# AMReX-Fluids/IAMR

Measured on AMD Instinct MI355X. Metric: cells-advanced/sec, higher is better.
Workload: dtype f64; 1 GPU; TaylorGreen 3D single level, one 256^3 box per GPU in a 1x1x1 arrangement (256x256x256 cells), periodic, nu=1e-4 cfl=0.7 Godunov_PLM be_cn_theta=0.5, full NavierStokes::advance per step

## Files before the change

iamr_amd/csrc/cabi.hip:

```cpp
#include "../../include/iamrx.h"
#include "operators.h"
#include "launch.h"
#include "amrns.h"
#include <string>
#include <cstring>
#include <vector>
#include <map>

using namespace iamrx;

struct iamrx_layout_s { LayoutP p; };
struct iamrx_mf_s { MultiFab mf; };

static thread_local std::string g_err;

#define IAMRX_TRY try {
#define IAMRX_CATCH                                                   \
    return 0; }                                                       \
    catch (const std::exception& e) { g_err = e.what(); return 1; }   \
    catch (...) { g_err = "unknown error"; return 2; }

static Geometry to_geom(const iamrx_geom* g)
{
    Geometry r;
// ... 102 lines not shown
            o[2] = cd.src_fab >= 0 ? local[cd.src_fab] : -1;
            o[3] = cd.dst_fab >= 0 ? local[cd.dst_fab] : -1;
            for (int d = 0; d < 3; ++d) { o[4 + d] = cd.region.lo[d]; o[7 + d] = cd.region.hi[d]; o[10 + d] = cd.shift[d]; }
            o[13] = (int)cd.buf_off; o[14] = 0; o[15] = 0;
        }
        ++n;
    };
    for (auto& cd : plan.local) emit(0, -1, cd);
    for (auto& kv : peers) {
        for (auto& cd : kv.second.pack) emit(1, kv.first, cd);
        for (auto& cd : kv.second.unpack) emit(2, kv.first, cd);
    }
    *ndesc = n;
    IAMRX_CATCH
}

int iamrx_host_abec_smoother_plan(int nboxes, const int* lo_hi, const iamrx_geom* g, const int lobc[3], const int hibc[3], int maxorder, int ncomp,
                                  int coef, int has_a, int has_cf, int finest, const int ngrow[4], int out[12])
{
    IAMRX_TRY
    if (nboxes < 1 || coef < 0 || coef > 2) throw Error("iamrx_host_abec_smoother_plan: at least one box; coef is 0 (stored), 1 (density) or 2 (uniform)");
    std::vector<BoxD> b(nboxes);
    AbecLevel lv;
    for (int i = 0; i < nboxes; ++i)
        for (int d = 0; d < 3; ++d) { b[i].lo[d] = lo_hi[6 * i + d]; b[i].hi[d] = lo_hi[6 * i + 3 + d]; lv.max_len[d] = std::max(lv.max_len[d], b[i].len(d)); }
    const DomainBC bc = to_bc(lobc, hibc, maxorder);
    lv.boxes = &b; lv.nlocal = nboxes; lv.ncomp = ncomp;
    lv.phi_ngrow = ngrow[0]; lv.rhs_ngrow = ngrow[1]; lv.sig_ngrow = ngrow[2]; lv.a_ngrow = ngrow[3];
    lv.sig = coef == 1; lv.b_uniform = coef == 2; lv.has_a = has_a != 0; lv.nbc = 1; lv.bcs = &bc; lv.has_cf = has_cf != 0; lv.finest = finest != 0;
    const AbecSmoothPlan p = abec_smooth_plan(to_geom(g), lv);
    const AbecColourForm& f = p.colour;
    const int v[12] = {(int)p.path, p.nw, p.nbr_splits, p.zero_first, (int)f.kernel, f.mode, f.np, f.maintain, f.allcf, f.wrap, f.walls_inkernel, f.zero_ok};
    std::copy(v, v + 12, out);
    IAMRX_CATCH
}

int iamrx_host_nodal_smoother_plan(int nboxes, const int* lo_hi, const iamrx_geom* g, const int lobc[3], const int hibc[3], int has_mask,
                                   int nodal_smoother, int bottom_smoother_only, int device_bottom, int nodal_sweeps, int coarsest, const int ngrow[2],
                                   int out[11])
{
    IAMRX_TRY
    if (nboxes < 1) throw Error("iamrx_host_nodal_smoother_plan: at least one box");
    std::vector<BoxD> b(nboxes);
    NodalLevel lv;
    for (int i = 0; i < nboxes; ++i)
        for (int d = 0; d < 3; ++d) { b[i].lo[d] = lo_hi[6 * i + d]; b[i].hi[d] = lo_hi[6 * i + 3 + d]; lv.max_len[d] = std::max(lv.max_len[d], b[i].len(d)); }
    DomainBC bc = to_bc(lobc, hibc, 2);
    for (int d = 0; d < 3; ++d) { if (bc.lo[d] == lo_inflow) bc.lo[d] = lo_neumann; if (bc.hi[d] == lo_inflow) bc.hi[d] = lo_neumann; }
    lv.boxes = &b; lv.nlocal = nboxes; lv.bc = &bc;
    lv.cor_ngrow = ngrow[0]; lv.rhs_ngrow = ngrow[1];
    lv.has_mask = has_mask != 0;
    lv.nodal_smoother = nodal_smoother; lv.bottom_smoother_only = bottom_smoother_only; lv.device_bottom = device_bottom; lv.nodal_sweeps = nodal_sweeps;
    lv.coarsest = coarsest != 0;
    const NodalSmoothPlan p = nodal_smooth_plan(to_geom(g), lv);
    const int v[11] = {(int)p.path, p.ngrow, p.wrap, p.refl, p.images, p.written_first, p.zero_start, p.par_fill, p.splits, (int)p.bottom, p.sweeps};
    std::copy(v, v + 11, out);
    IAMRX_CATCH
}

static hipEvent_t g_ev0 = nullptr, g_ev1 = nullptr;
int iamrx_timer_start(void)
{
    IAMRX_TRY
    if (!g_ev0) { IAMRX_HIP_CHECK(hipEventCreate(&g_ev0)); IAMRX_HIP_CHECK(hipEventCreate(&g_ev1)); }
    IAMRX_HIP_CHECK(hipEventRecord(g_ev0, Context::get().stream));
    IAMRX_CATCH
// ... 1463 lines not shown
```

iamr_amd/csrc/kernels.h:

```cpp
#pragma once
#include "core.h"
#include "mf.h"

namespace iamrx {

void launch_fill(double* p, size_t n, double v, hipStream_t s);
void launch_copy_plan(const CopyDesc* d, int nd, long maxpts, const FabD* src, const FabD* dst, int scomp, int dcomp, int nc, hipStream_t s, bool add = false);
void launch_pack(const CopyDesc* d, int nd, long maxpts, const FabD* src, double* buf, long pts_total, int scomp, int nc, hipStream_t s);
void launch_unpack(const CopyDesc* d, int nd, long maxpts, const FabD* dst, const double* buf, long pts_total, int dcomp, int nc, hipStream_t s, bool add = false);
void launch_copy_plan_w(const CopyDesc* d, const int2* w, int nw, const FabD* src, const FabD* dst, int scomp, int dcomp, int nc, hipStream_t s, bool add);
void launch_pack_w(const CopyDesc* d, const int2* w, int nw, const FabD* src, double* buf, long pts_total, int scomp, int nc, hipStream_t s);
void launch_unpack_w(const CopyDesc* d, const int2* w, int nw, const FabD* dst, const double* buf, long pts_total, int dcomp, int nc, hipStream_t s, bool add);
double reduce_norm0(const MultiFab& mf, int comp, int nc, int ng, bool global = false);
void reduce_norm0_comps(const MultiFab& mf, int comp, int nc, int ng, double* out, bool global = false);
void reduce_minmax(const MultiFab& mf, int comp, int ng, double& mn, double& mx, bool global = true);
double reduce_sum_unique(const MultiFab& mf, int comp, const Geometry& g, bool global = false);
void reduce_sum_integrated(const MultiFab& S, int rho_comp, int trac_comp, const MultiFab* cov, double out[3]);
void reduce_dots(int nout, const MultiFab* const* x, const MultiFab* const* y, int comp, int nc, const Geometry& g, double* out, bool local = false);
void reduce_dots_dev(int nout, const MultiFab* const* x, const MultiFab* const* y, int comp, int nc, const Geometry& g, double* d_out, bool local = false);
enum { PROBE_NODAL_GS4 = 0, PROBE_ABEC_GSRB = 1, PROBE_GOD_Z = 2, PROBE_PRED_Z = 3, PROBE_COUNT = 4 };
void kernel_probe_start(int which, long min_points, int stride);
void kernel_probe_stop(int which, double* total_ms, long* launches);
void kernel_probes_pause(bool on);
bool kernel_probe_begin(int which, long points);
// ... 51 lines not shown
    const DomainBC* bcs = nullptr;
    bool has_cf = false;
    bool finest = true;
};
AbecLevel abec_level(const AbecCoef& c, const MultiFab& phi, int rhs_ngrow, int nbc, const DomainBC* bcs, bool has_cf = false, bool finest = true);
struct AbecColourForm {
    enum Kernel { GENERAL, GSRB1, GSRB2, GSRB2_PER_COMP } kernel = GENERAL;
    int mode = 0;
    int np = 1;
    bool gen_mc = false;
    int gen_mode = 0;
    bool has_cf = false, maintain = false, allcf = false;
    bool wrap = false;
    bool walls_inkernel = false;
    bool zero_ok = false;
};
struct AbecSmoothPlan {
    enum Path { COLOUR, RB_BOX, RB_CF, RB_NBR, FUSED_SHELL } path = COLOUR;
    AbecColourForm colour;
    int nw = 16;
    bool nbr_splits = false;
    bool zero_first = false;
    int ncomp = 1, phi_ngrow = 1, rhs_ngrow = 0;
    bool sweep_kernel() const { return path == RB_BOX || path == RB_CF || path == RB_NBR; }
    bool made_for(const MultiFab& phi, const MultiFab& rhs) const { return phi.ncomp == ncomp && phi.ngrow == phi_ngrow && rhs.ngrow == rhs_ngrow; }
};
AbecSmoothPlan abec_smooth_plan(const Geometry& g, const AbecLevel& lv);
AbecColourForm abec_colour_form(const Geometry& g, const AbecLevel& lv, bool wrap = false, bool walls_inkernel = false);
void abec_gsrb(const Geometry& g, const AbecCoef& c, const AbecColourForm& f, MultiFab& phi, const MultiFab& rhs, int redblack, double omega,
               const DomainBC* bcs, int nbc, bool shell_only = false, bool phi_is_zero = false, const MultiFab* cfm = nullptr, const CfTab* cftab = nullptr);
bool abec_tail_ok(const Geometry& gF, const Layout& lF, const Geometry& gC, const Layout& lC, const AbecCoef& cF, const DomainBC* bcs, int nbc, int ncomp);
void abec_tail_solve(const Geometry& gF, const AbecCoef& cF, MultiFab& corF, const MultiFab& resF, const Geometry& gC, const AbecCoef& cC,
                     const DomainBC& bc, bool singular, double eps_rel, int maxiter, int nub, int nuf, int nu1, int nu2, double omega, int* d_iters);
bool abec_residual_reads_no_ghosts(const Geometry& g, const AbecCoef& c, const MultiFab& out, const MultiFab& phi, const MultiFab& rhs, bool restrict_form);
bool abec_resid_restrict_ok(const AbecCoef& c, const MultiFab& phi, const MultiFab& rhs);
void abec_resid_restrict(const Geometry& g, const AbecCoef& c, MultiFab& crse, const MultiFab& phi, const MultiFab& rhs);
void abec_gsrb_rb(const Geometry& g, const AbecCoef& c, const AbecSmoothPlan& p, const MultiFab& pin, MultiFab& pout, const MultiFab& rhs, double omega,
                  bool zero, const DomainBC* bcs = nullptr, int nbc = 0, const CfTab* cf = nullptr, bool acc = false);
void abec_gsrb_rb_nbr(const Geometry& g, const AbecCoef& c, const AbecSmoothPlan& p, MultiFab& pin, MultiFab& pout, const MultiFab& rhs, double omega,
                      bool zero, const DomainBC* bcs, int nbc, int sel = 0, hipStream_t on = nullptr, bool acc = false);
bool abec_gsrb_rb_ok(const Geometry& g, const AbecCoef& c, const MultiFab& phi, int nbc, const DomainBC* bcs = nullptr);
bool abec_gsrb_rb_cf_ok(const Geometry& g, const AbecCoef& c, const MultiFab& phi);
bool abec_gsrb_rb_nbr_ok(const Geometry& g, const AbecCoef& c, const MultiFab& phi, const MultiFab& rhs, int nbc, const DomainBC* bcs);
bool abec_gsrb_rb_nbr_level_ok(const Geometry& g, const Layout& l, int ncomp, bool sig_form, bool has_a, int nbc, const DomainBC* bcs);
void abec_gsrb_fused(const Geometry& g, const AbecCoef& c, const MultiFab& phi_in, MultiFab& phi_out, const MultiFab& rhs, double omega,
                     const DomainBC* bcs, int nbc);
void abec_residual(const Geometry& g, const AbecCoef& c, MultiFab& out, const MultiFab& phi, const MultiFab* rhs, double* norm_out = nullptr);
bool abec_bottom_device_ok(const Geometry& g, const Layout& l, const DomainBC* bcs, int nbc, int ncomp, bool cf = false);
void abec_bottom_solve(const Geometry& g, const AbecCoef& c, MultiFab& cor, const MultiFab& res, const DomainBC& bc, bool singular,
                       double eps_rel, int maxiter, int nub, int nuf, double omega, int* d_iters, const CfTab* cftab = nullptr);
void abec_apply_domain_bc(const Geometry& g, MultiFab& phi, const DomainBC& bc, bool inhomog, const MultiFab* bcval, int comp0 = 0, int ncomp = -1);
void abec_apply_domain_bc_percomp(const Geometry& g, MultiFab& phi, const DomainBC* bcs, int ncomp, bool inhomog, const MultiFab* bcval);
void cc_restrict(MultiFab& crse, const MultiFab& fine);
void cc_prolong_add(MultiFab& fine, const MultiFab& crse);
void face_avgdown(MultiFab& crse, const MultiFab& fine, int dir);
void abec_flux(const Geometry& g, const AbecCoef& c, const MultiFab& phi, MultiFab* const flux[3], MultiFab* const add_to[3]);
void mac_rhs(const Geometry& g, MultiFab& rhs, const MultiFab* const umac[3], const MultiFab* S);
void mac_bcoef(MultiFab* const b[3], const MultiFab& rho, int rho_comp, double scale);
void mac_divergence(const Geometry& g, MultiFab& div, const MultiFab* const umac[3]);

void godunov_extrap_vel_to_faces(const Geometry& g, const MultiFab& vel, const MultiFab* force, MultiFab* const umac[3],
                                 double dt, const BCRec* bc, bool use_forces_in_trans, int scheme = 0);
void godunov_compute_aofs(const Geometry& g, MultiFab& aofs, int acomp, const MultiFab& S, int ncomp, const MultiFab* force,
                          const MultiFab* divu, MultiFab* const umac[3], const int* iconserv, double dt, const BCRec* bc,
                          bool is_velocity, bool use_forces_in_trans, MultiFab* const edge_out[3], MultiFab* const flux_out[3], int scheme = 0);

// ... 73 lines not shown
```

iamr_amd/csrc/mlmg.h:

```cpp
#pragma once
#include <functional>
#include "mf.h"
#include "kernels.h"
#include <vector>
#include <memory>

namespace iamrx {

inline bool mg_stalled_at_floor(const std::vector<double>& hist, double r0, double target, bool fast)
{
    const size_t n = hist.size();
    if (n == 0 || !(hist[n - 1] <= 10.0 * target)) return false;
    if (n >= 4 && hist[n - 1] > 0.9 * hist[n - 4]) return true;
    if (!fast || n < 2) return false;
    const double last = hist[n - 1] / hist[n - 2];
    double best = 1.0, prev = r0;
    for (size_t i = 0; i + 1 < n; ++i) { if (prev > 0.0) best = std::min(best, hist[i] / prev); prev = hist[i]; }
    return last > 0.5 && best < 0.2;
}


struct MGOpts {
    int nu1 = 2, nu2 = 2, nuf = 8, nub = 0;
    int max_iters = 200;
// ... 79 lines not shown
public:
    CellMG(const Geometry& g, LayoutP layout, int ncomp, const DomainBC& bc, const MGOpts& o);
    void setScalars(double alpha, double beta) { m_alpha = alpha; m_beta = beta; }
    void setACoeffs(const MultiFab* a) { m_a0 = a; }
    void setBCoeffs(const MultiFab* const b[3]) { for (int d = 0; d < 3; ++d) m_b0[d] = b[d]; }
    void setBCoeffsFromCell(const MultiFab* sig, int comp, double scale) { m_sig = sig; m_sig_comp = comp; m_sig_scale = scale; }
    void setTensor(bool t) { m_tensor = t; }
    void setTensorEta(bool t) { m_tensor_eta = t; }
    void setDomainBCs(const DomainBC* bcs, int n) { m_bcn.assign(bcs, bcs + n); }
    void setCoarseFineBC(const MultiFab* crse, const Geometry& cgeom, int ratio) { m_cf = true; m_crse = crse; m_cgeom = cgeom; m_ratio = ratio; }
    void prepare();
    void prepareBoundary();
    void fillBoundaryData(MultiFab& phi);
    MGStats solve(MultiFab& phi, const MultiFab& rhs, double rtol, double atol);
    void apply(MultiFab& out, MultiFab& phi);
    void fluxes(MultiFab& phi, MultiFab* const flux[3], MultiFab* const add_to[3]);
    int nlevels() const { return (int)m_lev.size(); }
    AbecCoef coef(int l) const;
    AbecCoef smoother_coef(int l) const;
    const Geometry& geom(int l) const { return m_lev[l].g; }
    void applyBC(int l, MultiFab& phi, bool inhomog, const MultiFab* bcval, bool corners = true);
    void smooth(int l, bool skip_fill, bool cf_ghosts_current = false, bool sol_is_zero = false);
    void smooth_n(int l, int nsweeps, bool skip_first_fill, bool sol_is_zero = false, MultiFab* acc = nullptr);
    void vcycle(MGStats& st);
    MultiFab& res(int l) { return m_lev[l].res; }
    MultiFab& cor(int l) { return m_lev[l].cor; }

private:
    struct Level : MGLevel {
        MultiFab a, b[3];
        MultiFab cor, res, rescor;
        MultiFab buf;
        AbecSmoothPlan plan;
        MultiFab cfm;
        CfTab cftab;
    };
    int bicgstab(int l, MultiFab& sol, const MultiFab& rhs, double eps_rel, double eps_abs, int& niters);
    void bottom_solve(MGStats& st);
    template <class Sweep> void pingpong(MultiFab& sol, MultiFab& buf, int nsweeps, bool sol_is_zero, MultiFab* acc, Sweep sweep);
    bool tail_fused() const;
    void cf_bcval(MultiFab& bcval);
    void prepare_cf(int l);
    void subtract_mean(int l, MultiFab& mf);
    Geometry m_g;
    int m_ncomp;
    std::vector<DomainBC> m_bcn;
    MGOpts m_o;
    double m_alpha = 0.0, m_beta = 1.0;
    const MultiFab* m_a0 = nullptr;
    const MultiFab* m_b0[3] = {nullptr, nullptr, nullptr};
    bool m_buni = false;
    bool m_buni_coarse = false;
    double m_bu[3] = {0.0, 0.0, 0.0};
    const MultiFab* m_sig = nullptr;
    int m_sig_comp = 0;
    double m_sig_scale = 1.0;
    bool m_tensor = false;
    bool m_tensor_eta = false;
    bool m_singular = false;
    bool m_bottom_dev = false;
    MultiFab* m_acc = nullptr;
    bool m_acc_done = false;
    bool m_bottom_direct = false;
    const double* m_dB = nullptr;
    std::shared_ptr<double> m_dBh;
    int m_dN = 0;
// ... 58 lines not shown
```

iamr_amd/csrc/mlmg.hip:

```cpp
#include "mlmg.h"
#include "krylov.h"
#include "launch.h"
#include <chrono>
#include <cmath>

namespace iamrx {

void parallel_copy(MultiFab& dst, const MultiFab& src, int scomp, int dcomp, int nc, int src_ng, int dst_ng, const Geometry* periodic_geom, bool add);

CycleTimer& cycle_timer() { static CycleTimer t; return t; }

long mg_agglomeration_cells() { return (long)tune("MG_AGGLOMERATE_CELLS", 2097152.0); }

bool mg_agglomerate_level(const Layout& c)
{
    if (c.replicated || c.total_cells() > mg_agglomeration_cells()) return false;
    if (Context::get().comm->nranks > 1) return true;
    return c.boxes.size() > 1 && tune("MG_AGG_SINGLE_RANK", 1) != 0;
}

bool mg_slab_level(const Geometry& g, const Layout& l, int min_width, bool slab_problem)
{
    if (!slab_problem && tune("MG_SLAB", 0) == 0) return false;
    if (!g.periodic[1] || g.domain.lo[1] != 0 || g.domain.hi[1] != 1) return false;
// ... 178 lines not shown
    }
    m_bottom_dev = m_o.device_bottom && m_dd_sweeps == 0 && !m_tensor && !m_o.bottom_smoother_only &&
                   abec_bottom_device_ok(m_lev.back().g, *m_lev.back().layout, m_bcn.data(), (int)m_bcn.size(), m_ncomp, m_cf);
    for (int l = 0; l < nl; ++l) {
        Level& L = m_lev[l];
        L.cor.define(L.layout, cell_type(), m_ncomp, (l == 0 && m_nbr) ? 2 : 1);
        L.res.define(L.layout, cell_type(), m_ncomp, (l == 0 && m_nbr) ? 1 : 0);
        L.rescor.define(L.layout, cell_type(), m_ncomp, 0);
        prepare_cf(l);
        if (l > 0) {
            AbecCoef fc = coef(l - 1);
            if (L.agg) L.tmp_d.define(L.dist, cell_type(), m_ncomp, 0);
            if (L.slab) L.vres.define(L.virt, cell_type(), m_ncomp, 0);
            auto coarsen_into = [&](MultiFab& dst, IndexType t, int nc, const std::function<void(MultiFab&)>& op) {
                MultiFab dist_arr, v;
                if (L.agg) dist_arr.define(L.dist, t, nc, 0);
                if (L.slab) v.define(L.virt, t, nc, 0);
                mg_restrict_to(L, dst, dist_arr, v, op);
            };
            if (m_a0) {
                L.a.define(L.layout, cell_type(), 1, 0);
                coarsen_into(L.a, cell_type(), 1, [&](MultiFab& c) { cc_restrict(c, *fc.a); });
            }
            for (int d = 0; d < 3; ++d) {
                MultiFab b3;
                const MultiFab* fb = fc.b[d];
                if (l == 1 && m_tensor_eta && !m_buni_coarse) { b3.define(m_lev[0].layout, face_type(d), 3, 0); tensor_bcoef(b3, *fc.b[d], d); fb = &b3; }
                L.b[d].define(L.layout, face_type(d), fb->ncomp, 0);
                coarsen_into(L.b[d], face_type(d), fb->ncomp, [&](MultiFab& c) { face_avgdown(c, *fb, d); });
            }
        }
        L.plan = abec_smooth_plan(L.g, abec_level(coef(l), L.cor, L.res.ngrow, (int)m_bcn.size(), m_bcn.data(), m_cf, l == 0));
    }
    bottom_direct_prepare();
}


void CellMG::applyBC(int l, MultiFab& phi, bool inhomog, const MultiFab* bcval, bool corners)
{
    if (phi.ngrow > 1) { const int one[3] = {1, 1, 1}; phi.FillBoundary(m_lev[l].g, 0, phi.ncomp, one); }
    else phi.FillBoundary(m_lev[l].g);
    if (m_bcn.size() == 1) abec_apply_domain_bc(m_lev[l].g, phi, m_bcn[0], inhomog, bcval);
    else if (m_ncomp <= 3 && (int)m_bcn.size() >= m_ncomp)
        abec_apply_domain_bc_percomp(m_lev[l].g, phi, m_bcn.data(), m_ncomp, inhomog, bcval);
    else
        for (int n = 0; n < m_ncomp; ++n) abec_apply_domain_bc(m_lev[l].g, phi, m_bcn[n], inhomog, bcval, n, 1);
    if (m_cf) cf_fill_ghosts(phi, m_lev[l].cfm, m_lev[l].cftab, inhomog, bcval, m_tensor);
    if (m_tensor && corners) {
        if (m_bcn.size() == 1) fill_tensor_corners(m_lev[l].g, phi, m_bcn[0], inhomog, bcval);
        else for (int n = 0; n < m_ncomp; ++n) fill_tensor_corners(m_lev[l].g, phi, m_bcn[n], inhomog, bcval, n, 1);
    }
}

void CellMG::cf_bcval(MultiFab& bcval)
{
    if (!m_cf) return;
    LayoutP cl = m_lev[0].layout->coarsened(m_ratio);
    MultiFab cpatch(cl, cell_type(), m_ncomp, 1);
    cpatch.setVal(0.0);
    if (m_crse) parallel_copy(cpatch, *m_crse, 0, 0, m_ncomp, 0, 1, &m_cgeom, false);
    cf_interp_bndry(bcval, cpatch, m_lev[0].cfm, m_ratio);
    if (m_tensor) cf_interp_edges(bcval, cpatch, m_lev[0].cfm, m_ratio, m_cgeom);
}

static double dd_omega()
{
// ... 272 lines not shown
    MultiFab b(L.layout, cell_type(), m_ncomp, 0);
    MultiFab::Copy(b, L.res, 0, 0, m_ncomp, 0);
    if (m_singular) subtract_mean(l, b);
    int nit = 0;
    int ret = bicgstab(l, L.cor, b, m_o.bottom_reltol, -1.0, nit);
    st.bottom_iters_total += nit;
    if (ret != 0) {
        L.cor.setVal(0.0);
        smooth_n(l, m_o.nuf, true);
    }
    const int nn = (ret == 0) ? m_o.nub : m_o.nuf;
    smooth_n(l, nn, false);
}

bool CellMG::tail_fused() const
{
    const int nl = (int)m_lev.size();
    if (nl < 2 || !m_bottom_dev || m_cf || m_dd_sweeps > 0 || m_o.nu1 <= 0) return false;
    const Level& F = m_lev[nl - 2];
    const Level& C = m_lev[nl - 1];
    if (C.agg || C.slab || F.slab || F.plan.path == AbecSmoothPlan::FUSED_SHELL) return false;
    AbecCoef cF = coef(nl - 2);
    return abec_tail_ok(F.g, *F.layout, C.g, *C.layout, cF, m_bcn.data(), (int)m_bcn.size(), m_ncomp);
}

void CellMG::vcycle(MGStats& st)
{
    const int nl = (int)m_lev.size();
    m_lev[0].res_filled = false;
    const bool tail = tail_fused();
    const int nsm = tail ? nl - 2 : nl - 1;
    for (int l = 0; l < nsm; ++l) {
        Level& L = m_lev[l];
        const bool z = m_o.nu1 > 0 && L.plan.zero_first;
        if (!z) L.cor.setVal(0.0);
        smooth_n(l, m_o.nu1, true, z);
        const AbecCoef cl = coef(l);
        if (m_cf || !abec_residual_reads_no_ghosts(L.g, cl, L.rescor, L.cor, L.res, true)) applyBC(l, L.cor, false, nullptr);
        Level& C = m_lev[l + 1];
        mg_restrict_to(C, C.res, C.tmp_d, C.vres, [&](MultiFab& target) {
            if (abec_resid_restrict_ok(cl, L.cor, L.res)) abec_resid_restrict(L.g, cl, target, L.cor, L.res);
            else {
                level_residual(L.g, cl, L.rescor, L.cor, &L.res);
                cc_restrict(target, L.rescor);
            }
        });
    }
    if (tail) {
        Level& F = m_lev[nl - 2];
        Level& C = m_lev[nl - 1];
        const int maxiter = krylov_maxiter(m_o.bottom_maxiter, C.layout->total_cells() * m_ncomp);
        abec_tail_solve(F.g, smoother_coef(nl - 2), F.cor, F.res, C.g, smoother_coef(nl - 1), m_bcn[0], m_singular, m_o.bottom_reltol, maxiter, m_o.nub, m_o.nuf,
                        m_o.nu1, m_o.nu2, m_o.omega, mg_bottom_iters_dev());
    } else
    bottom_solve(st);
    for (int l = nsm - 1; l >= 0; --l) {
        Level& L = m_lev[l];
        cc_prolong_add(L.cor, mg_correction_of(m_lev[l + 1], m_lev[l + 1].cor, 0));
        smooth_n(l, m_o.nu2, false, false, l == 0 ? m_acc : nullptr);
    }
}

void CellMG::fillBoundaryData(MultiFab& phi)
{
    const Geometry& g0 = m_lev[0].g;
    if (m_cf || !(g0.periodic[0] && g0.periodic[1] && g0.periodic[2])) {
        MultiFab bcval(m_lev[0].layout, cell_type(), m_ncomp, 1);
        MultiFab::Copy(bcval, phi, 0, 0, m_ncomp, 1);
        cf_bcval(bcval);
        applyBC(0, phi, true, &bcval);
    } else applyBC(0, phi, true, nullptr);
}

void CellMG::apply(MultiFab& out, MultiFab& phi)
{
    fillBoundaryData(phi);
    level_residual(m_lev[0].g, coef(0), out, phi, nullptr);
}

void CellMG::fluxes(MultiFab& phi, MultiFab* const flux[3], MultiFab* const add_to[3])
{
    abec_flux(m_lev[0].g, coef(0), phi, flux, add_to);
}

MGStats CellMG::solve(MultiFab& phi, const MultiFab& rhs_in, double rtol, double atol)
{
    ProfScope ps_prof_("cmg_solve");
    auto& ctx = Context::get();
    MGStats st;
    st.nlevels = (int)m_lev.size();
// ... 86 lines not shown
```

iamr_amd/lib.py:

```python
import ctypes as C
import os
import numpy as np

_HERE = os.path.dirname(os.path.abspath(__file__))
LIB_PATH = os.path.join(_HERE, "libiamrx.so")
_lib = None


class IamrxError(RuntimeError):
    pass


class Geom(C.Structure):
    _fields_ = [("dom_lo", C.c_int * 3), ("dom_hi", C.c_int * 3), ("prob_lo", C.c_double * 3),
                ("prob_hi", C.c_double * 3), ("periodic", C.c_int * 3)]

    @staticmethod
    def make(n, prob_lo=(0.0, 0.0, 0.0), prob_hi=(1.0, 1.0, 1.0), periodic=(1, 1, 1)):
        g = Geom()
        g.dom_lo = (C.c_int * 3)(0, 0, 0)
        g.dom_hi = (C.c_int * 3)(*[int(n[d]) - 1 for d in range(3)])
        g.prob_lo = (C.c_double * 3)(*prob_lo)
        g.prob_hi = (C.c_double * 3)(*prob_hi)
        g.periodic = (C.c_int * 3)(*periodic)
# ... 346 lines not shown

    def InitRHS(self, rhs):
        check(lib().iamrx_syncreg_init_rhs(self.h, rhs.h))

    def __del__(self):
        try:
            if self.h:
                lib().iamrx_syncreg_destroy(self.h)
                self.h = None
        except Exception:
            pass


def average_down(fine, crse, scomp=0, ncomp=None, ratio=2):
    check(lib().iamrx_average_down(fine.h, crse.h, scomp, crse.ncomp if ncomp is None else ncomp, ratio))


SMOOTHER_PATHS = ("COLOUR", "RB_BOX", "RB_CF", "RB_NBR", "FUSED_SHELL")
SMOOTHER_KERNELS = ("general", "gsrb1", "gsrb2", "gsrb2_per_comp")


def host_abec_smoother_plan(geom, boxes, ncomp=1, coef=1, has_a=False, has_cf=False, finest=True, ngrow=(1, 0, 1, 0), lobc=(0, 0, 0), hibc=(0, 0, 0),
                            maxorder=3):
    arr = (C.c_int * (6 * len(boxes)))(*[int(v) for lo, hi in boxes for v in tuple(lo) + tuple(hi)])
    out = (C.c_int * 12)()
    check(lib().iamrx_host_abec_smoother_plan(len(boxes), arr, C.byref(geom), i3(lobc), i3(hibc), int(maxorder), int(ncomp), int(coef), int(has_a),
                                              int(has_cf), int(finest), (C.c_int * 4)(*[int(v) for v in ngrow]), out))
    keys = ("path", "nw", "nbr_splits", "zero_first", "kernel", "mode", "np", "maintain", "allcf", "wrap", "walls_inkernel", "zero_ok")
    d = dict(zip(keys, out[:]))
    d["path"], d["kernel"] = SMOOTHER_PATHS[d["path"]], SMOOTHER_KERNELS[d["kernel"]]
    return d


NODAL_SMOOTHER_PATHS = ("JACOBI", "COLOUR8", "SMALL", "GS4", "GSR")
NODAL_BOTTOM_KINDS = ("NONE", "SMOOTHER_ONLY", "DEVICE_PERIODIC", "DEVICE_GENERAL", "HOST_KRYLOV")


def host_nodal_smoother_plan(geom, boxes, has_mask=False, nodal_smoother=0, bottom_smoother_only=False, device_bottom=True, nodal_sweeps=2,
                             coarsest=False, ngrow=(4, 4), lobc=(0, 0, 0), hibc=(0, 0, 0)):
    arr = (C.c_int * (6 * len(boxes)))(*[int(v) for lo, hi in boxes for v in tuple(lo) + tuple(hi)])
    out = (C.c_int * 11)()
    check(lib().iamrx_host_nodal_smoother_plan(len(boxes), arr, C.byref(geom), i3(lobc), i3(hibc), int(has_mask), int(nodal_smoother),
                                               int(bottom_smoother_only), int(device_bottom), int(nodal_sweeps), int(coarsest),
                                               (C.c_int * 2)(*[int(v) for v in ngrow]), out))
    keys = ("path", "ngrow", "wrap", "refl", "images", "written_first", "zero_start", "par_fill", "splits", "bottom", "sweeps")
    d = dict(zip(keys, out[:]))
    d["path"], d["bottom"] = NODAL_SMOOTHER_PATHS[d["path"]], NODAL_BOTTOM_KINDS[d["bottom"]]
    return d


TURB_FIELDS = ("FTX", "TAT", "FPX", "FPY", "FPZ", "FAX", "FAY", "FAZ", "FPXX", "FPXY", "FPXZ", "FPYX", "FPYY", "FPYZ", "FPZX", "FPZY", "FPZZ")


def host_turb_modes(prob_lo, prob_hi, nmodes=4, mode_start=0, div_free=1):
    lo, hi = (C.c_double * 3)(*[float(v) for v in prob_lo]), (C.c_double * 3)(*[float(v) for v in prob_hi])
    M = C.c_int()
    check(lib().iamrx_host_turb_modes(lo, hi, int(nmodes), int(mode_start), int(div_free), 0, C.byref(M), None, None))
    k = np.zeros((M.value, 3), dtype=np.int32)
    d = np.zeros((M.value, 17))
    check(lib().iamrx_host_turb_modes(lo, hi, int(nmodes), int(mode_start), int(div_free), M.value, C.byref(M), k.ctypes.data_as(C.POINTER(C.c_int)),
                                      d.ctypes.data_as(C.POINTER(C.c_double))))
    return k, d


def _turb_table(kxyz, data):
    k = np.ascontiguousarray(kxyz, dtype=np.int32).reshape(-1, 3)
# ... 273 lines not shown
```

include/iamrx.h:

```cpp
#ifndef IAMRX_H
#define IAMRX_H
#include <stddef.h>

#ifdef __cplusplus
extern "C" {
#endif

typedef struct iamrx_layout_s* iamrx_layout;
typedef struct iamrx_fluxreg_s* iamrx_fluxreg;
typedef struct iamrx_mf_s* iamrx_mf;
typedef struct iamrx_ns_s* iamrx_ns;
typedef struct iamrx_syncreg_s* iamrx_syncreg;
typedef struct iamrx_amr_s* iamrx_amr;

typedef struct iamrx_geom {
    int dom_lo[3], dom_hi[3];
    double prob_lo[3], prob_hi[3];
    int periodic[3];
} iamrx_geom;

typedef struct iamrx_mg_opts {
    int nu1, nu2, nuf, nub;
    int max_iters, bottom_maxiter;
    double bottom_reltol;
// ... 51 lines not shown
int iamrx_layout_create(int nboxes, const int* lo_hi , const int* owner_rank,
                        iamrx_layout* out);
int iamrx_layout_coalesced_boxes(iamrx_layout l, int* nboxes, int* lo_hi );
int iamrx_layout_destroy(iamrx_layout l);
int iamrx_layout_nlocal(iamrx_layout l, int* nlocal);
int iamrx_layout_local_box(iamrx_layout l, int local_idx, int lo_hi[6], int* global_idx);
int iamrx_layout_owners(iamrx_layout l, int* owners );
int iamrx_mf_create(iamrx_layout l, const int type[3] , int ncomp, int ngrow, iamrx_mf* out);
int iamrx_mf_destroy(iamrx_mf m);
int iamrx_mf_info(iamrx_mf m, int* ncomp, int* ngrow, int type[3], int* nlocal);
int iamrx_mf_fab_box(iamrx_mf m, int local_idx, int lo_hi[6]);
int iamrx_mf_dev_ptr(iamrx_mf m, int local_idx, double** p);
int iamrx_mf_to_host(iamrx_mf m, int local_idx, double* dst);
int iamrx_mf_from_host(iamrx_mf m, int local_idx, const double* src);
int iamrx_mf_setval(iamrx_mf m, double v);
int iamrx_mf_copy(iamrx_mf dst, iamrx_mf src, int scomp, int dcomp, int ncomp, int ngrow);
int iamrx_mf_fill_boundary(iamrx_mf m, const iamrx_geom* g);
int iamrx_mf_fill_physbc(iamrx_mf m, const iamrx_geom* g, int scomp, int ncomp, const int* bcrec, const double* extdir_lo,
                         const double* extdir_hi);
int iamrx_mf_norm0(iamrx_mf m, int comp, int ncomp, int ngrow, double* out);
int iamrx_mf_norm0_comps(iamrx_mf m, int comp, int ncomp, int ngrow, int form, double* out);
int iamrx_mf_minmax(iamrx_mf m, int comp, int ngrow, double* mn, double* mx);
int iamrx_mf_dot(const iamrx_geom* g, const int lobc[3], const int hibc[3], iamrx_mf x0, iamrx_mf y0, iamrx_mf x1, iamrx_mf y1, int comp,
                 int ncomp, int on_device, double out[2]);
int iamrx_mf_sum_unique(const iamrx_geom* g, const int lobc[3], const int hibc[3], iamrx_mf m, int comp, double* out);

int iamrx_host_fill_plan(int nboxes, const int* lo_hi, const int* owner, int rank, const int type[3], int ngrow, const iamrx_geom* g,
                         int max_desc, int* desc, int* ndesc);
int iamrx_host_fill_plan_wall_ext(int nboxes, const int* lo_hi, const int* owner, int rank, const int type[3], int ngrow, const iamrx_geom* g,
                                  int wall_ext, int max_desc, int* desc, int* ndesc);

int iamrx_host_abec_smoother_plan(int nboxes, const int* lo_hi, const iamrx_geom* g, const int lobc[3], const int hibc[3], int maxorder, int ncomp,
                                  int coef, int has_a, int has_cf, int finest, const int ngrow[4], int out[12]);
int iamrx_host_nodal_smoother_plan(int nboxes, const int* lo_hi, const iamrx_geom* g, const int lobc[3], const int hibc[3], int has_mask,
                                   int nodal_smoother, int bottom_smoother_only, int device_bottom, int nodal_sweeps, int coarsest, const int ngrow[2],
                                   int out[11]);

int iamrx_abec_gsrb(const iamrx_geom* g, double alpha, double beta, iamrx_mf a , iamrx_mf bx, iamrx_mf by, iamrx_mf bz,
                    iamrx_mf phi, iamrx_mf rhs, int redblack, double omega, const int lobc[3], const int hibc[3], int maxorder);
int iamrx_abec_form(const iamrx_geom* g, int coef, iamrx_mf rho, int rho_comp, double scale, const double bu[3], double beta, int op,
                    iamrx_mf phi, iamrx_mf rhs, iamrx_mf out, double omega, const int lobc[3], const int hibc[3], int maxorder);
int iamrx_abec_gsrb_sweep(const iamrx_geom* g, double alpha, double beta, iamrx_mf a , iamrx_mf bx, iamrx_mf by, iamrx_mf bz,
                          iamrx_mf phi, iamrx_mf rhs, double omega, const int lobc[3], const int hibc[3], int maxorder, int fused);
int iamrx_abec_residual(const iamrx_geom* g, double alpha, double beta, iamrx_mf a, iamrx_mf bx, iamrx_mf by, iamrx_mf bz,
                        iamrx_mf out, iamrx_mf phi, iamrx_mf rhs, int tensor);
int iamrx_cc_restrict(iamrx_mf crse, iamrx_mf fine);
int iamrx_cc_prolong_add(iamrx_mf fine, iamrx_mf crse);
int iamrx_face_avgdown(iamrx_mf crse, iamrx_mf fine, int dir);
int iamrx_abec_solve(const iamrx_geom* g, double alpha, double beta, iamrx_mf a, iamrx_mf bx, iamrx_mf by, iamrx_mf bz,
                     iamrx_mf phi, iamrx_mf rhs, const int lobc[3], const int hibc[3], double rtol, double atol,
                     const iamrx_mg_opts* o, int tensor, iamrx_mg_stats* st);

int iamrx_mlmg_mac_solve(const iamrx_geom* g, iamrx_mf umac_x, iamrx_mf umac_y, iamrx_mf umac_z, iamrx_mf rho, int rho_comp,
                         iamrx_mf S , iamrx_mf mac_phi, double rhs_scale, const int lobc[3], const int hibc[3],
                         double mac_tol, double mac_abs_tol, const iamrx_mg_opts* o, iamrx_mg_stats* st);
int iamrx_mlmg_mac_solve_cf(const iamrx_geom* g, iamrx_mf umac_x, iamrx_mf umac_y, iamrx_mf umac_z, iamrx_mf rho, int rho_comp,
                            iamrx_mf S , iamrx_mf mac_phi, double rhs_scale, const int lobc[3], const int hibc[3],
                            iamrx_mf crse_phi, const iamrx_geom* cgeom, int ratio, double mac_tol, double mac_abs_tol,
                            const iamrx_mg_opts* o, iamrx_mg_stats* st);
int iamrx_mac_sync_solve(const iamrx_geom* g, iamrx_fluxreg mac_reg, iamrx_mf rho_half, double dt, iamrx_layout fine, int ratio,
                         iamrx_mf ucorr_x, iamrx_mf ucorr_y, iamrx_mf ucorr_z, iamrx_mf mac_sync_phi, const int lobc[3], const int hibc[3],
                         double mac_sync_tol, double mac_abs_tol, const iamrx_mg_opts* o, iamrx_mg_stats* st);
int iamrx_mac_divergence(const iamrx_geom* g, iamrx_mf div, iamrx_mf umac_x, iamrx_mf umac_y, iamrx_mf umac_z);

#define IAMRX_GODUNOV_PLM 0
#define IAMRX_GODUNOV_PPM 1
// ... 218 lines not shown
```

Measured before the change: 492.1 million cells/s.

## Fuse coarse MG legs into single tiled smoother+restrict/prolong kernels

Adds a kernel that, on small periodic single-box coarse multigrid levels, runs the whole down leg (nu1 red-black GSRB sweeps from zero, residual, restriction) or up leg (prolongation add plus nu2 sweeps) in one launch. It uses 16^3 shared-memory tiles with redundant halo computation. This replaces many small launches and ghost fills on coarse levels, which are dominated by launch overhead. The cost is redundant halo work and a more restrictive eligibility path that has to match the existing smoother's numerics.

```diff
diff --git a/iamr_amd/csrc/cabi.hip b/iamr_amd/csrc/cabi.hip
--- a/iamr_amd/csrc/cabi.hip
+++ b/iamr_amd/csrc/cabi.hip
@@ -158,6 +158,26 @@
     const AbecColourForm& f = p.colour;
     const int v[12] = {(int)p.path, p.nw, p.nbr_splits, p.zero_first, (int)f.kernel, f.mode, f.np, f.maintain, f.allcf, f.wrap, f.walls_inkernel, f.zero_ok};
     std::copy(v, v + 12, out);
+    IAMRX_CATCH
+}
+
+int iamrx_host_abec_leg_plan(int nboxes, const int* lo_hi, const iamrx_geom* g, const int lobc[3], const int hibc[3], int maxorder, int ncomp,
+                             int coef, int has_a, int has_cf, int finest, const int ngrow[4], int level, int nu1, int nu2, int slab_transition,
+                             int agg_transition, int out[9])
+{
+    IAMRX_TRY
+    if (nboxes < 1 || coef < 0 || coef > 2) throw Error("iamrx_host_abec_leg_plan: at least one box; coef is 0 (stored), 1 (density) or 2 (uniform)");
+    std::vector<BoxD> b(nboxes);
+    AbecLevel lv;
+    for (int i = 0; i < nboxes; ++i)
+        for (int d = 0; d < 3; ++d) { b[i].lo[d] = lo_hi[6 * i + d]; b[i].hi[d] = lo_hi[6 * i + 3 + d]; lv.max_len[d] = std::max(lv.max_len[d], b[i].len(d)); }
+    const DomainBC bc = to_bc(lobc, hibc, maxorder);
+    lv.boxes = &b; lv.nlocal = nboxes; lv.ncomp = ncomp;
+    lv.phi_ngrow = ngrow[0]; lv.rhs_ngrow = ngrow[1]; lv.sig_ngrow = ngrow[2]; lv.a_ngrow = ngrow[3];
+    lv.sig = coef == 1; lv.b_uniform = coef == 2; lv.has_a = has_a != 0; lv.nbc = 1; lv.bcs = &bc; lv.has_cf = has_cf != 0; lv.finest = finest != 0;
+    const AbecLegPlan p = abec_leg_plan(to_geom(g), lv, level, nu1, nu2, slab_transition != 0, agg_transition != 0);
+    const int v[9] = {p.on ? 1 : 0, p.tile_down[0], p.tile_down[1], p.tile_down[2], p.tile_up[0], p.tile_up[1], p.tile_up[2], p.halo_down, p.halo_up};
+    std::copy(v, v + 9, out);
     IAMRX_CATCH
 }
 
diff --git a/iamr_amd/csrc/k_abec_legs.hip b/iamr_amd/csrc/k_abec_legs.hip
--- /dev/null
+++ b/iamr_amd/csrc/k_abec_legs.hip
@@ -0,0 +1,244 @@
+#include "kernels.h"
+#include <algorithm>
+
+namespace iamrx {
+
+constexpr int LEG_NT = 1024;
+constexpr int LEG_CELLS = LEG_R * LEG_R * LEG_R;
+static_assert(LEG_R == 16 && LEG_CELLS == 4 * LEG_NT, "a thread owns four cells of the region: two x-pairs, eight planes apart");
+
+struct LegArgs {
+    FabD rhs, A, bx, by, bz;
+    FabD buf;
+    FabD crs;
+    FabD cor;
+    int lo[3], n[3], t[3];
+    int halo, npass;
+    double alpha, dhx, dhy, dhz, omega;
+    double bu[3];
+};
+
+template <int BMODE, bool HASA, bool DOWN>
+__global__ void __launch_bounds__(LEG_NT) k_abec_leg(const LegArgs g)
+{
+    __shared__ double sh[LEG_CELLS];
+    __shared__ double shr[LEG_CELLS];
+    const int t = (int)threadIdx.x, px = t & 7, ry = (t >> 3) & (LEG_R - 1), rzb = t >> 7;
+    const int H = g.halo;
+    const int tb[3] = {(int)blockIdx.x, (int)blockIdx.y, (int)blockIdx.z};
+    int t0[3], t1[3], o[3];
+#pragma unroll
+    for (int d = 0; d < 3; ++d) {
+        t0[d] = g.lo[d] + tb[d] * g.t[d];
+        t1[d] = min(t0[d] + g.t[d] - 1, g.lo[d] + g.n[d] - 1);
+        o[d] = t0[d] - H;
+    }
+    auto image = [&](int d, int v) { int m = (v - g.lo[d]) % g.n[d]; if (m < 0) m += g.n[d]; return g.lo[d] + m; };
+    auto away = [&](int d, int v) { return max(max(t0[d] - v, v - t1[d]), 0); };
+    const int gy = o[1] + ry, wy = image(1, gy), dy = away(1, gy);
+
+    const int sred = (gy + o[2] + rzb) & 1;
+    const int at0 = 2 * px + LEG_R * (ry + LEG_R * rzb);
+    unsigned dpk = 0;
+#define IAMRX_LEG_AT(q, c) (at0 + (sred ^ (c)) + 8 * LEG_R * LEG_R * (q))
+#define IAMRX_LEG_DIST(q, c) ((int)((dpk >> (8 * (2 * (q) + (c)))) & 255u))
+    double p[2][2], w[2][2], aa[2][2];
+    double cxl[2], cxc[2], cxr[2];
+    double cym[2][2], cyp[2][2], czm[2][2], czp[2][2];
+    double rr[2][2];
+#pragma unroll
+    for (int q = 0; q < 2; ++q) {
+        const int rz = rzb + 8 * q, gz = o[2] + rz, wz = image(2, gz), dz = away(2, gz);
+        cxl[q] = cxc[q] = cxr[q] = 0.0;
+        if (BMODE == 0 && dy + dz + min(away(0, o[0] + 2 * px), away(0, o[0] + 2 * px + 1)) <= H) {
+            const int wx0 = image(0, o[0] + 2 * px);
+            cxl[q] = g.bx(wx0, wy, wz, 0); cxc[q] = g.bx(wx0 + 1, wy, wz, 0); cxr[q] = g.bx(wx0 + 2, wy, wz, 0);
+        }
+#pragma unroll
+        for (int c = 0; c < 2; ++c) {
+            const int x = 2 * px + (sred ^ c), gx = o[0] + x, wx = image(0, gx);
+            const int dist = min(away(0, gx) + dy + dz, 255);
+            dpk |= (unsigned)dist << (8 * (2 * q + c));
+            p[q][c] = 0.0; w[q][c] = 0.0; aa[q][c] = 0.0; rr[q][c] = 0.0;
+            cym[q][c] = cyp[q][c] = czm[q][c] = czp[q][c] = 0.0;
+            if (dist <= H) {
+                rr[q][c] = g.rhs(wx, wy, wz, 0);
+                if (HASA) aa[q][c] = g.A(wx, wy, wz, 0);
+                if (BMODE == 0) {
+                    cym[q][c] = g.by(wx, wy, wz, 0); cyp[q][c] = g.by(wx, wy + 1, wz, 0);
+                    czm[q][c] = g.bz(wx, wy, wz, 0); czp[q][c] = g.bz(wx, wy, wz + 1, 0);
+                }
+                if (!DOWN) { p[q][c] = g.buf(wx, wy, wz, 0); w[q][c] = g.crs(wx >> 1, wy >> 1, wz >> 1, 0); }
+            }
+        }
+    }
+#pragma unroll
+    for (int q = 0; q < 2; ++q)
+#pragma unroll
+        for (int c = 0; c < 2; ++c) {
+            if (IAMRX_LEG_DIST(q, c) <= H) {
+                if (!DOWN) p[q][c] = p[q][c] + w[q][c];
+                if (HASA) aa[q][c] = g.alpha * aa[q][c];
+                double bxm, bxp, bym, byp, bzm, bzp;
+                if (BMODE == 0) {
+                    bxm = (sred ^ c) ? cxc[q] : cxl[q]; bxp = (sred ^ c) ? cxr[q] : cxc[q];
+                    bym = cym[q][c]; byp = cyp[q][c]; bzm = czm[q][c]; bzp = czp[q][c];
+                } else { bxm = bxp = g.bu[0]; bym = byp = g.bu[1]; bzm = bzp = g.bu[2]; }
+                const double gamma = aa[q][c] + g.dhx * (bxm + bxp) + g.dhy * (bym + byp) + g.dhz * (bzm + bzp);
+                const double g_m_d = gamma - (g.dhx * (bxm * 0.0 + bxp * 0.0) + g.dhy * (bym * 0.0 + byp * 0.0) + g.dhz * (bzm * 0.0 + bzp * 0.0));
+                w[q][c] = g.omega / g_m_d;
+                shr[IAMRX_LEG_AT(q, c)] = rr[q][c];
+            }
+            sh[IAMRX_LEG_AT(q, c)] = p[q][c];
+        }
+    __syncthreads();
+
+    auto around = [&](int q, int c, double mate, double& pxm, double& pxp, double& pym, double& pyp, double& pzm, double& pzp) {
+        const double* at = sh + IAMRX_LEG_AT(q, c);
+        const bool left = !(sred ^ c);
+        const double po = at[left ? -1 : 1];
+        pxm = left ? po : mate; pxp = left ? mate : po;
+        pym = at[-LEG_R]; pyp = at[LEG_R];
+        pzm = at[-LEG_R * LEG_R]; pzp = at[LEG_R * LEG_R];
+    };
+    auto coefs = [&](int q, int c, double& bxm, double& bxp, double& bym, double& byp, double& bzm, double& bzp) {
+        if (BMODE == 0) { const bool right = sred ^ c; bxm = right ? cxc[q] : cxl[q]; bxp = right ? cxr[q] : cxc[q]; bym = cym[q][c]; byp = cyp[q][c]; bzm = czm[q][c]; bzp = czp[q][c]; }
+        else { bxm = bxp = g.bu[0]; bym = byp = g.bu[1]; bzm = bzp = g.bu[2]; }
+    };
+    const int reach = DOWN ? g.npass + 1 : g.npass;
+#define IAMRX_LEG_PASS(C, ZERO, pass)                                                                                              \
+    {                                                                                                                              \
+        _Pragma("unroll") for (int q = 0; q < 2; ++q)                                                                              \
+            if (IAMRX_LEG_DIST(q, C) + (pass) <= reach) {                                                                          \
+                double pxm = 0.0, pxp = 0.0, pym = 0.0, pyp = 0.0, pzm = 0.0, pzp = 0.0, bxm, bxp, bym, byp, bzm, bzp;             \
+                if (!(ZERO)) around(q, C, p[q][1 - C], pxm, pxp, pym, pyp, pzm, pzp);                                              \
+                coefs(q, C, bxm, bxp, bym, byp, bzm, bzp);                                                                         \
+                const int at = IAMRX_LEG_AT(q, C);                                                                                 \
+                const double pc = (ZERO) ? 0.0 : p[q][C];                                                                          \
+                const double gamma = (HASA ? aa[q][C] : 0.0) + g.dhx * (bxm + bxp) + g.dhy * (bym + byp) + g.dhz * (bzm + bzp);    \
+                const double rho = g.dhx * (bxm * pxm + bxp * pxp) + g.dhy * (bym * pym + byp * pyp) + g.dhz * (bzm * pzm + bzp * pzp); \
+                const double res = shr[at] - (gamma * pc - rho);                                                                   \
+                const double pn = pc + w[q][C] * res;                                                                              \
+                p[q][C] = pn;                                                                                                      \
+                sh[at] = pn;                                                                                                       \
+            }                                                                                                                      \
+        __syncthreads();                                                                                                           \
+    }
+    if (DOWN) {
+        IAMRX_LEG_PASS(0, true, 1)
+        IAMRX_LEG_PASS(1, false, 2)
+    }
+    for (int pass = DOWN ? 3 : 1; pass <= g.npass; pass += 2) {
+        IAMRX_LEG_PASS(0, false, pass)
+        IAMRX_LEG_PASS(1, false, pass + 1)
+    }
+#undef IAMRX_LEG_PASS
+
+    if (!DOWN) {
+#pragma unroll
+        for (int q = 0; q < 2; ++q)
+#pragma unroll
+            for (int c = 0; c < 2; ++c)
+                if (IAMRX_LEG_DIST(q, c) == 0) g.cor(o[0] + 2 * px + (sred ^ c), gy, o[2] + rzb + 8 * q, 0) = p[q][c];
+        return;
+    }
+#pragma unroll
+    for (int q = 0; q < 2; ++q)
+#pragma unroll
+        for (int c = 0; c < 2; ++c)
+            if (IAMRX_LEG_DIST(q, c) == 0) {
+                double pxm, pxp, pym, pyp, pzm, pzp, bxm, bxp, bym, byp, bzm, bzp;
+                around(q, c, p[q][1 - c], pxm, pxp, pym, pyp, pzm, pzp);
+                coefs(q, c, bxm, bxp, bym, byp, bzm, bzp);
+                const int at = IAMRX_LEG_AT(q, c);
+                const double p0 = p[q][c];
+                const double ax = HASA ? aa[q][c] * p0 : 0.0;
+                const double y = ax
+                    - g.dhx * (bxp * (pxp - p0) - bxm * (p0 - pxm))
+                    - g.dhy * (byp * (pyp - p0) - bym * (p0 - pym))
+                    - g.dhz * (bzp * (pzp - p0) - bzm * (p0 - pzm));
+                shr[at] = shr[at] - y;
+                g.buf(o[0] + 2 * px + (sred ^ c), gy, o[2] + rzb + 8 * q, 0) = p0;
+            }
+    __syncthreads();
+    const int ncx = (t1[0] - t0[0] + 1) >> 1, ncy = (t1[1] - t0[1] + 1) >> 1, ncz = (t1[2] - t0[2] + 1) >> 1;
+    if (t < ncx * ncy * ncz) {
+        const int I = t % ncx, J = (t / ncx) % ncy, K = t / (ncx * ncy);
+        double s = 0.0;
+        for (int kr = 0; kr < 2; ++kr)
+            for (int jr = 0; jr < 2; ++jr) {
+                const int at = H + 2 * I + LEG_R * (H + 2 * J + jr + LEG_R * (H + 2 * K + kr));
+                s += shr[at];
+                s += shr[at + 1];
+            }
+        g.crs((t0[0] >> 1) + I, (t0[1] >> 1) + J, (t0[2] >> 1) + K, 0) = 0.125 * s;
+    }
+#undef IAMRX_LEG_AT
+#undef IAMRX_LEG_DIST
+}
+
+AbecLegPlan abec_leg_plan(const Geometry& g, const AbecLevel& lv, int level, int nu1, int nu2, bool slab_transition, bool agg_transition)
+{
+    AbecLegPlan p;
+    p.halo_down = 2 * nu1; p.halo_up = 2 * nu2;
+    if (tune("MG_LEGS", 1) == 0 || level < 1 || lv.finest) return p;
+    if (lv.ncomp != 1 || lv.b_ncomp != 1 || lv.tensor || lv.tensor_eta || lv.has_cf || lv.sig || slab_transition || agg_transition) return p;
+    if (!(g.periodic[0] && g.periodic[1] && g.periodic[2]) || !lv.boxes || lv.boxes->size() != 1 || lv.nlocal != 1) return p;
+    if (nu1 < 1 || nu2 < 1 || LEG_R - 2 * p.halo_down < 2 || LEG_R - 2 * p.halo_up < 2) return p;
+    const BoxD& b = (*lv.boxes)[0];
+    for (int d = 0; d < 3; ++d)
+        if (b.lo[d] != g.domain.lo[d] || b.hi[d] != g.domain.hi[d] || (b.lo[d] & 1) || (b.len(d) & 1) || b.len(d) < 2) return p;
+    if ((double)b.npts() > tune("MG_LEGS_MAX_CELLS", 262144.0)) return p;
+    p.on = true;
+    p.mode = (lv.b_uniform && tune("ABEC_SIG", 1) != 0) ? 2 : 0;
+    for (int d = 0; d < 3; ++d) {
+        p.tile_down[d] = std::min(LEG_R - 2 * p.halo_down, b.len(d));
+        p.tile_up[d] = std::min(LEG_R - 2 * p.halo_up, b.len(d));
+    }
+    return p;
+}
+
+template <bool DOWN>
+static void leg_launch(const Geometry& g, const AbecCoef& c, const AbecLegPlan& p, LegArgs& a, const MultiFab& rhs, int nu, double omega)
+{
+    IAMRX_ASSERT(p.on && rhs.nlocal() == 1 && rhs.ncomp == 1 && !c.sig && !c.tensor && !c.tensor_eta);
+    const bool has_a = c.a && c.alpha != 0.0;
+    const BoxD& b = rhs.layout->lbox(0);
+    const int* tile = DOWN ? p.tile_down : p.tile_up;
+    a.rhs = rhs.h_tab[0];
+    a.A = has_a ? c.a->h_tab[0] : rhs.h_tab[0];
+    a.bx = c.b[0]->h_tab[0]; a.by = c.b[1]->h_tab[0]; a.bz = c.b[2]->h_tab[0];
+    dim3 grid;
+    for (int d = 0; d < 3; ++d) { a.lo[d] = b.lo[d]; a.n[d] = b.len(d); a.t[d] = tile[d]; }
+    grid.x = (a.n[0] + a.t[0] - 1) / a.t[0]; grid.y = (a.n[1] + a.t[1] - 1) / a.t[1]; grid.z = (a.n[2] + a.t[2] - 1) / a.t[2];
+    a.halo = a.npass = 2 * nu;
+    IAMRX_ASSERT(a.halo == (DOWN ? p.halo_down : p.halo_up) && a.t[0] + 2 * a.halo <= LEG_R && a.t[1] + 2 * a.halo <= LEG_R && a.t[2] + 2 * a.halo <= LEG_R);
+    a.alpha = c.alpha; a.omega = omega;
+    a.dhx = c.beta / (g.dx[0] * g.dx[0]); a.dhy = c.beta / (g.dx[1] * g.dx[1]); a.dhz = c.beta / (g.dx[2] * g.dx[2]);
+    for (int d = 0; d < 3; ++d) a.bu[d] = c.bu[d];
+    hipStream_t s = Context::get().stream;
+#define IAMRX_LEG(M, HA) hipLaunchKernelGGL((k_abec_leg<M, HA, DOWN>), grid, dim3(LEG_NT), 0, s, a)
+    if (p.mode == 2) { if (has_a) IAMRX_LEG(2, true); else IAMRX_LEG(2, false); }
+    else { if (has_a) IAMRX_LEG(0, true); else IAMRX_LEG(0, false); }
+#undef IAMRX_LEG
+}
+
+void abec_leg_down(const Geometry& g, const AbecCoef& c, const AbecLegPlan& p, MultiFab& buf, const MultiFab& rhs, MultiFab& crse_rhs, int nu1, double omega)
+{
+    if (rhs.nlocal() == 0) return;
+    IAMRX_ASSERT(buf.layout.get() == rhs.layout.get() && crse_rhs.nlocal() == 1 && crse_rhs.ncomp == 1);
+    LegArgs a;
+    a.buf = buf.h_tab[0]; a.crs = crse_rhs.h_tab[0]; a.cor = buf.h_tab[0];
+    leg_launch<true>(g, c, p, a, rhs, nu1, omega);
+}
+
+void abec_leg_up(const Geometry& g, const AbecCoef& c, const AbecLegPlan& p, MultiFab& cor, const MultiFab& buf, const MultiFab& rhs, const MultiFab& crse_cor, int nu2, double omega)
+{
+    if (rhs.nlocal() == 0) return;
+    IAMRX_ASSERT(buf.layout.get() == rhs.layout.get() && cor.layout.get() == rhs.layout.get() && crse_cor.nlocal() == 1 && crse_cor.ncomp == 1);
+    LegArgs a;
+    a.buf = buf.h_tab[0]; a.crs = crse_cor.h_tab[0]; a.cor = cor.h_tab[0];
+    leg_launch<false>(g, c, p, a, rhs, nu2, omega);
+}
+
+}
diff --git a/iamr_amd/csrc/kernels.h b/iamr_amd/csrc/kernels.h
--- a/iamr_amd/csrc/kernels.h
+++ b/iamr_amd/csrc/kernels.h
@@ -107,6 +107,17 @@
 bool abec_tail_ok(const Geometry& gF, const Layout& lF, const Geometry& gC, const Layout& lC, const AbecCoef& cF, const DomainBC* bcs, int nbc, int ncomp);
 void abec_tail_solve(const Geometry& gF, const AbecCoef& cF, MultiFab& corF, const MultiFab& resF, const Geometry& gC, const AbecCoef& cC,
                      const DomainBC& bc, bool singular, double eps_rel, int maxiter, int nub, int nuf, int nu1, int nu2, double omega, int* d_iters);
+constexpr int LEG_R = 16;
+struct AbecLegPlan {
+    bool on = false;
+    int mode = 0;
+    int tile_down[3] = {0, 0, 0}, tile_up[3] = {0, 0, 0};
+    int halo_down = 0, halo_up = 0;
+};
+AbecLegPlan abec_leg_plan(const Geometry& g, const AbecLevel& lv, int level, int nu1, int nu2, bool slab_transition, bool agg_transition);
+void abec_leg_down(const Geometry& g, const AbecCoef& c, const AbecLegPlan& p, MultiFab& buf, const MultiFab& rhs, MultiFab& crse_rhs, int nu1, double omega);
+void abec_leg_up(const Geometry& g, const AbecCoef& c, const AbecLegPlan& p, MultiFab& cor, const MultiFab& buf, const MultiFab& rhs, const MultiFab& crse_cor, int nu2,
+                 double omega);
 bool abec_residual_reads_no_ghosts(const Geometry& g, const AbecCoef& c, const MultiFab& out, const MultiFab& phi, const MultiFab& rhs, bool restrict_form);
 bool abec_resid_restrict_ok(const AbecCoef& c, const MultiFab& phi, const MultiFab& rhs);
 void abec_resid_restrict(const Geometry& g, const AbecCoef& c, MultiFab& crse, const MultiFab& phi, const MultiFab& rhs);
diff --git a/iamr_amd/csrc/mlmg.h b/iamr_amd/csrc/mlmg.h
--- a/iamr_amd/csrc/mlmg.h
+++ b/iamr_amd/csrc/mlmg.h
@@ -135,6 +135,7 @@
         MultiFab cor, res, rescor;
         MultiFab buf;
         AbecSmoothPlan plan;
+        AbecLegPlan legs;
         MultiFab cfm;
         CfTab cftab;
     };
diff --git a/iamr_amd/csrc/mlmg.hip b/iamr_amd/csrc/mlmg.hip
--- a/iamr_amd/csrc/mlmg.hip
+++ b/iamr_amd/csrc/mlmg.hip
@@ -234,6 +234,19 @@
         }
         L.plan = abec_smooth_plan(L.g, abec_level(coef(l), L.cor, L.res.ngrow, (int)m_bcn.size(), m_bcn.data(), m_cf, l == 0));
     }
+    for (int l = 0; l < nl; ++l) {
+        Level& L = m_lev[l];
+        L.legs = AbecLegPlan();
+        if (l < 1 || l + 1 >= nl || m_dd_sweeps > 0) continue;
+        const Level& C = m_lev[l + 1];
+        L.legs = abec_leg_plan(L.g, abec_level(coef(l), L.cor, L.res.ngrow, (int)m_bcn.size(), m_bcn.data(), m_cf, false), l, m_o.nu1, m_o.nu2,
+                               L.slab || C.slab, C.agg);
+    }
+    if (nl >= 2 && m_lev[nl - 2].legs.on && tail_fused()) m_lev[nl - 2].legs.on = false;
+    for (int l = 0; l < nl; ++l) {
+        Level& L = m_lev[l];
+        if (L.legs.on && (!L.buf.defined() || L.buf.ngrow != L.cor.ngrow)) L.buf.define(L.layout, cell_type(), m_ncomp, L.cor.ngrow);
+    }
     bottom_direct_prepare();
 }
 
@@ -572,6 +585,10 @@
     const int nsm = tail ? nl - 2 : nl - 1;
     for (int l = 0; l < nsm; ++l) {
         Level& L = m_lev[l];
+        if (L.legs.on) {
+            abec_leg_down(L.g, coef(l), L.legs, L.buf, L.res, m_lev[l + 1].res, m_o.nu1, m_o.omega);
+            continue;
+        }
         const bool z = m_o.nu1 > 0 && L.plan.zero_first;
         if (!z) L.cor.setVal(0.0);
         smooth_n(l, m_o.nu1, true, z);
@@ -596,6 +613,10 @@
     bottom_solve(st);
     for (int l = nsm - 1; l >= 0; --l) {
         Level& L = m_lev[l];
+        if (L.legs.on) {
+            abec_leg_up(L.g, smoother_coef(l), L.legs, L.cor, L.buf, L.res, m_lev[l + 1].cor, m_o.nu2, m_o.omega);
+            continue;
+        }
         cc_prolong_add(L.cor, mg_correction_of(m_lev[l + 1], m_lev[l + 1].cor, 0));
         smooth_n(l, m_o.nu2, false, false, l == 0 ? m_acc : nullptr);
     }
diff --git a/iamr_amd/lib.py b/iamr_amd/lib.py
--- a/iamr_amd/lib.py
+++ b/iamr_amd/lib.py
@@ -402,6 +402,17 @@
     return d
 
 
+def host_abec_leg_plan(geom, boxes, level, nu1=2, nu2=2, ncomp=1, coef=0, has_a=False, has_cf=False, ngrow=(1, 0, 0, 0), lobc=(0, 0, 0), hibc=(0, 0, 0),
+                       maxorder=3, slab_transition=False, agg_transition=False):
+    arr = (C.c_int * (6 * len(boxes)))(*[int(v) for lo, hi in boxes for v in tuple(lo) + tuple(hi)])
+    out = (C.c_int * 9)()
+    check(lib().iamrx_host_abec_leg_plan(len(boxes), arr, C.byref(geom), i3(lobc), i3(hibc), int(maxorder), int(ncomp), int(coef), int(has_a),
+                                         int(has_cf), int(level == 0), (C.c_int * 4)(*[int(v) for v in ngrow]), int(level), int(nu1), int(nu2),
+                                         int(slab_transition), int(agg_transition), out))
+    v = out[:]
+    return dict(legs=bool(v[0]), tile_down=tuple(v[1:4]), tile_up=tuple(v[4:7]), halo_down=v[7], halo_up=v[8])
+
+
 NODAL_SMOOTHER_PATHS = ("JACOBI", "COLOUR8", "SMALL", "GS4", "GSR")
 NODAL_BOTTOM_KINDS = ("NONE", "SMOOTHER_ONLY", "DEVICE_PERIODIC", "DEVICE_GENERAL", "HOST_KRYLOV")
 
diff --git a/include/iamrx.h b/include/iamrx.h
--- a/include/iamrx.h
+++ b/include/iamrx.h
@@ -107,6 +107,9 @@
 
 int iamrx_host_abec_smoother_plan(int nboxes, const int* lo_hi, const iamrx_geom* g, const int lobc[3], const int hibc[3], int maxorder, int ncomp,
                                   int coef, int has_a, int has_cf, int finest, const int ngrow[4], int out[12]);
+int iamrx_host_abec_leg_plan(int nboxes, const int* lo_hi, const iamrx_geom* g, const int lobc[3], const int hibc[3], int maxorder, int ncomp,
+                             int coef, int has_a, int has_cf, int finest, const int ngrow[4], int level, int nu1, int nu2, int slab_transition,
+                             int agg_transition, int out[9]);
 int iamrx_host_nodal_smoother_plan(int nboxes, const int* lo_hi, const iamrx_geom* g, const int lobc[3], const int hibc[3], int has_mask,
                                    int nodal_smoother, int bottom_smoother_only, int device_bottom, int nodal_sweeps, int coarsest, const int ngrow[2],
                                    int out[11]);
```

After: 500.0 million cells/s (median of 6 runs). 1.6% higher.
